# lucidrains/magvit2-pytorch

Hardware: NVIDIA H100
Metric: video-frames/sec tokenize+decode, 17x128x128 bf16 (higher is better)
Workload: dtype bf16

## Files before the change

### magvit2_pytorch_b200/csrc/tc_slab.cu

```cuda
#include "common.cuh"
#include "tc_common.cuh"
#include <cuda.h>
#include <algorithm>
#include <type_traits>
#include <mutex>
#include <map>
#include <vector>
#include <string.h>

namespace mv2 {

struct alignas(64) SlabParams {
  CUtensorMap amap;
  CUtensorMap hmap;
  CUtensorMap wmap;
  CUtensorMap wmap2;
  int kt, kh, kw, pt, ph, pw;
  int st;
  int hist_T;
  int Ci, kchunks, row_bytes;
  int B, T, H, W, Co;
  int mw, pitch, slab_h, slab_bytes, slab_stride;
  int bn, n_tiles_n, tiles_w, tiles_h, total_tiles;
  int slab_stages, w_stages;
  int tpw;
  TcEpi epi;
  int dtype;
  CUtensorMap w1map;
  const float* bias1;
  const float* se_wk;
  float se_bk;
  float* se_ws;
  CUtensorMap amap_odd;
  int dn_e_off;
  int dn_aoff[6];
  int dn_lower;
  int h_stride;
  CUtensorMap ymap;
  CUtensorMap rmap;
};

__host__ __device__ constexpr bool slab_tma_epi(int mode) {
  return mode == EPI_PLAIN || mode == EPI_PLAIN_RES || mode == EPI_GEGLU || mode == EPI_DOWN_SPACE;
}
__host__ __device__ constexpr int slab_out_box_ch(int mode, int bn, int es) {
  return (mode == EPI_GEGLU ? bn / 2 : bn) < 128 / es ? (mode == EPI_GEGLU ? bn / 2 : bn) : 128 / es;
}

__host__ __device__ __forceinline__ void slab_frame_of(const SlabParams& p, int slot, int& b, int& t) {
  const int ptc = p.pt > 0 ? (p.pt + p.st - 1) / p.st : 0;
  const int n_cheap = ptc < p.T ? ptc : p.T, n_full = p.T - n_cheap;
  const int full_slots = p.B * n_full;
  if (slot < full_slots) { b = slot / n_full; t = n_cheap + slot - b * n_full; }
  else { const int r = slot - full_slots; const int level = r / p.B; b = r - level * p.B; t = n_cheap - 1 - level; }
}
__host__ __device__ __forceinline__ int slab_tile_of_cta(const SlabParams& p, int k, int cta, int grid) {
  const int tile = k * grid + ((k & 1) ? grid - 1 - cta : cta);
  return tile < p.total_tiles ? tile : -1;
}
__device__ __forceinline__ int slab_tile_of(const SlabParams& p, int k) { return slab_tile_of_cta(p, k, blockIdx.x, gridDim.x); }

struct TileCoord { int b, t, h0, w0, n0; };
__host__ __device__ __forceinline__ TileCoord decode_tile(const SlabParams& p, int tile) {
  TileCoord c;
  const int nt = tile % p.n_tiles_n; tile /= p.n_tiles_n;
  const int tw = tile % p.tiles_w; tile /= p.tiles_w;
  const int th = tile % p.tiles_h; tile /= p.tiles_h;
  slab_frame_of(p, tile, c.b, c.t);
  c.h0 = th * 16;
  c.w0 = tw * 8 * p.mw;
  c.n0 = nt * p.bn;
  return c;
}

struct SlabSmem { uint32_t sbias, stage0, lpart, accstg, hbuf, end, rbar, otile, rtile; };
__host__ __device__ __forceinline__ SlabSmem slab_smem_layout(const SlabParams& p, uint32_t bar0, bool fused, uint32_t es) {
  SlabSmem m = {};
  m.sbias = (bar0 + 8 * (2 * p.slab_stages + 2 * p.w_stages) + 15) & ~15u;
  m.stage0 = m.sbias + (uint32_t)(p.n_tiles_n * p.bn) * 4 * (fused ? 3 : 1);
  if (fused) {
    m.lpart = m.stage0;
    m.hbuf = (m.lpart + 2048 + 1023u) & ~1023u;
    m.otile = m.hbuf + (uint32_t)p.h_stride;
    m.end = m.otile + 2u * p.mw * 64 * p.bn * es;
    return m;
  }
  m.accstg = m.stage0 + 8 * 2048;
  m.end = m.accstg + 2u * p.mw * 64 * (p.bn + 4) * 4;
  m.rbar = m.stage0;
  m.otile = (m.rbar + 32 + 1023u) & ~1023u;
  m.rtile = m.otile + 2u * p.mw * 64 * p.bn * es;
  const uint32_t tiles_end = m.rtile + (p.epi.res ? 2u * p.mw * 64 * p.bn * es : 0u);
  if (tiles_end > m.end) m.end = tiles_end;
  return m;
}

template <typename T, int MODE, int BN, int ACT>
__device__ __forceinline__ void slab_epi_mtile(const SlabParams& p, const float (&acc)[BN / 2], const TileCoord& c,
                                               const float* sbias, uint32_t ot, uint32_t rt, int wq, int lane, bool relu) {
  constexpr int ES = sizeof(T);
  constexpr int CB = slab_out_box_ch(MODE, BN, ES);
  constexpr uint32_t RB = CB * ES, BOX = 64 * RB, SWZ = (RB / 16 - 1) << 4;
  const uint32_t m0 = 16 * wq + (lane >> 2), q4 = (lane & 3) * 2 * ES;
  auto at = [&](int col, uint32_t m) {
    const uint32_t off = m * RB + (uint32_t)(col % CB) * ES + q4;
    return (uint32_t)(col / CB) * BOX + (off ^ ((off >> 3) & SWZ));
  };
  auto st2 = [](uint32_t a, float v0, float v1) {
    if constexpr (ES == 4) asm volatile("st.shared.v2.f32 [%0], {%1, %2};" ::"r"(a), "f"(v0), "f"(v1) : "memory");
    else asm volatile("st.shared.b32 [%0], %1;" ::"r"(a), "r"(pack2<T>(v0, v1)) : "memory");
  };
  const float* os = (MODE == EPI_PLAIN || MODE == EPI_PLAIN_RES) && p.epi.oscale ? p.epi.oscale + (int64_t)c.b * p.Co : nullptr;
  const float rs = MODE == EPI_PLAIN_RES && p.epi.mode == 2 ? 0.70710678118654752440f : 1.f;
  if (MODE == EPI_GEGLU) {
#pragma unroll
    for (int g = 0; g < BN / 16; ++g) {
      const int n = c.n0 + 16 * g + 2 * (lane & 3);
      const float2 bx = *reinterpret_cast<const float2*>(sbias + n), bg = *reinterpret_cast<const float2*>(sbias + n + 8);
#pragma unroll
      for (int hr = 0; hr < 2; ++hr) {
        const float* xv = &acc[8 * g + 2 * hr];
        const float* gv = &acc[8 * g + 4 + 2 * hr];
        const float v0 = gelu_fast(gv[0] + bg.x) * (xv[0] + bx.x);
        const float v1 = gelu_fast(gv[1] + bg.y) * (xv[1] + bx.y);
        st2(ot + at(8 * g, m0 + 8 * hr), v0, v1);
      }
    }
  } else {
#pragma unroll
    for (int g = 0; g < BN / 8; ++g) {
      const int col = 8 * g, n = c.n0 + col + 2 * (lane & 3);
      const float2 b = *reinterpret_cast<const float2*>(sbias + n);
      float o0 = 1.f, o1 = 1.f;
      if (os) { o0 = n < p.Co ? os[n] : 0.f; o1 = n + 1 < p.Co ? os[n + 1] : 0.f; }
#pragma unroll
      for (int hr = 0; hr < 2; ++hr) {
        float v0 = acc[4 * g + 2 * hr], v1 = acc[4 * g + 2 * hr + 1];
        if (os) { v0 *= o0; v1 *= o1; }
        v0 = act_ct<ACT>(v0 + b.x, relu);
        v1 = act_ct<ACT>(v1 + b.y, relu);
        const uint32_t a = at(col, m0 + 8 * hr);
        if (MODE == EPI_PLAIN_RES) {
          float2 rf;
          if constexpr (ES == 4) {
            asm volatile("ld.shared.v2.f32 {%0, %1}, [%2];" : "=f"(rf.x), "=f"(rf.y) : "r"(rt + a) : "memory");
          } else {
            uint32_t r;
            asm volatile("ld.shared.b32 %0, [%1];" : "=r"(r) : "r"(rt + a) : "memory");
            rf = unpack2<T>(r);
          }
          v0 = (v0 + rf.x) * rs;
          v1 = (v1 + rf.y) * rs;
        }
        st2(ot + a, v0, v1);
      }
    }
  }
}
template <typename T, int MODE, int BN, int ACT, int MWMAX>
__device__ __forceinline__ void slab_epi_fragment(const SlabParams& p, const float (&acc)[MWMAX][BN / 2], const TileCoord& c,
                                                  const float* sbias, uint32_t ot, uint32_t rt, int wq, int lane, bool relu) {
  constexpr uint32_t MTILE = (MODE == EPI_GEGLU ? BN / 2 : BN) * 64 * (int)sizeof(T);
#pragma unroll
  for (int j = 0; j < MWMAX; ++j) {
    if (j >= p.mw) break;
    slab_epi_mtile<T, MODE, BN, ACT>(p, acc[j], c, sbias, ot + j * MTILE, rt + j * MTILE, wq, lane, relu);
  }
}

constexpr int SLAB_PRODUCER_REGS = 40, SLAB_CONSUMER_REGS = 232;
template <typename T, int MODE, int BN>
__device__ __forceinline__ void tc_slab_body(const SlabParams& p) {
  constexpr int MWMAX = BN >= 32 ? 128 / BN : 4;
  constexpr int KC1 = BN >= 64 ? BN / 64 : 1;
  constexpr bool TMA_STORE = slab_tma_epi(MODE) || MODE == EPI_FUSED_RU;
  extern __shared__ uint8_t smem_raw[];
  const uint32_t smem_base = (smem_u32(smem_raw) + 1023u) & ~1023u;
  const int warp = threadIdx.x >> 5, lane = threadIdx.x & 31;
  const uint32_t row_bytes = p.row_bytes;
  const uint32_t bk = row_bytes / (uint32_t)sizeof(T);
  const uint32_t w_tile = p.bn * row_bytes;
  const uint32_t w_bytes = w_tile * p.tpw;
  const uint32_t slab0 = smem_base;
  const uint32_t wst0 = smem_base + p.slab_stages * p.slab_stride;
  const uint32_t bar0 = wst0 + p.w_stages * w_bytes;
  const uint32_t slab_full = bar0, slab_empty = slab_full + 8 * p.slab_stages;
  const uint32_t w_full = slab_empty + 8 * p.slab_stages, w_empty = w_full + 8 * p.w_stages;
  const SlabSmem L = slab_smem_layout(p, bar0, MODE == EPI_FUSED_RU, (uint32_t)sizeof(T));
  auto gen = [&](uint32_t u) { return smem_raw + (u - smem_u32(smem_raw)); };
  float* sbias = reinterpret_cast<float*>(gen(L.sbias));
  const uint32_t nbias = (uint32_t)(p.n_tiles_n * p.bn);
  const uint32_t stage0 = L.stage0;

  if (threadIdx.x == 0) {
    for (int s = 0; s < p.slab_stages; ++s) { mbar_init(slab_full + 8 * s, 1); mbar_init(slab_empty + 8 * s, 8); }
    for (int s = 0; s < p.w_stages; ++s) { mbar_init(w_full + 8 * s, 1); mbar_init(w_empty + 8 * s, 8); }
    if (MODE == EPI_PLAIN_RES)
      for (int g = 0; g < 2; ++g) { mbar_init(L.rbar + 8 * g, 1); mbar_init(L.rbar + 16 + 8 * g, 4); }
    fence_barrier_init();
  }
  if (warp == 0 && lane == 0) {
    tma_prefetch_desc(&p.amap);
    if (MODE == EPI_DOWN_SPACE) tma_prefetch_desc(&p.amap_odd);
    else if (p.hist_T > 0) tma_prefetch_desc(&p.hmap);
  }
  if (warp == 2 && lane == 0) {
    tma_prefetch_desc(&p.wmap); tma_prefetch_desc(&p.wmap2);
    if (MODE == EPI_FUSED_RU) tma_prefetch_desc(&p.w1map);
  }
  if (TMA_STORE && warp == 1 && lane == 0) {
    tma_prefetch_desc(&p.ymap);
    if (MODE == EPI_PLAIN_RES) tma_prefetch_desc(&p.rmap);
  }
  if (warp >= 4) {
    const int nb = p.n_tiles_n * p.bn;
    for (int i = threadIdx.x - 128; i < nb; i += 256) sbias[i] = (p.epi.bias && i < p.Co) ? p.epi.bias[i] : 0.f;
    if (MODE == EPI_FUSED_RU)
      for (int i = threadIdx.x - 128; i < nb; i += 256) {
        sbias[nb + i] = (p.bias1 && i < p.Co) ? p.bias1[i] : 0.f;
        sbias[2 * nb + i] = i < p.Co ? p.se_wk[i] : 0.f;
      }
  }
  __syncthreads();
  pdl_wait();
  pdl_launch_dependents();

  const int taps2d = p.kh * p.kw;

  if (warp < 4) {
    setmaxnreg_dec<SLAB_PRODUCER_REGS>();
    if (warp == 0) {
      if (MODE == EPI_DOWN_SPACE) {
        if (lane == 0) {
          uint32_t s = 0, ph = 0;
          for (int tk = 0, tile; (tile = slab_tile_of(p, tk)) >= 0; ++tk) {
            const TileCoord c = decode_tile(p, tile);
            for (int kc = 0; kc < p.kchunks; ++kc) {
              mbar_wait(slab_empty + 8 * s, ph ^ 1);
              mbar_expect_tx(slab_full + 8 * s, p.slab_bytes);
              tma_load_5d(slab0 + s * p.slab_stride, &p.amap_odd, slab_full + 8 * s, kc * bk, c.w0 - 1, c.h0 - 1, c.t, c.b);
              tma_load_5d(slab0 + s * p.slab_stride + p.dn_e_off, &p.amap, slab_full + 8 * s, kc * bk, c.w0 - 1, c.h0, c.t, c.b);
              if (++s == (uint32_t)p.slab_stages) { s = 0; ph ^= 1; }
            }
          }
        }
      } else
      if (lane == 0) {
        uint32_t s = 0, ph = 0;
        for (int tk = 0, tile; (tile = slab_tile_of(p, tk)) >= 0; ++tk) {
          const TileCoord c = decode_tile(p, tile);
          const int dt0 = max(0, p.pt - c.t * p.st - p.hist_T);
          for (int dt = dt0; dt < p.kt; ++dt)
            for (int kc = 0; kc < p.kchunks; ++kc) {
              mbar_wait(slab_empty + 8 * s, ph ^ 1);
              mbar_expect_tx(slab_full + 8 * s, p.slab_bytes);
              const int ti = c.t * p.st + dt - p.pt;
              tma_load_5d(slab0 + s * p.slab_stride, ti >= 0 ? &p.amap : &p.hmap, slab_full + 8 * s, kc * bk, c.w0 - p.pw,
                          c.h0 - p.ph, ti >= 0 ? ti : ti + p.hist_T, c.b);
              if (++s == (uint32_t)p.slab_stages) { s = 0; ph ^= 1; }
            }
        }
      }
    } else if (warp == 1) {
      if (MODE == EPI_PLAIN_RES && lane == 0) {
        constexpr int CB = slab_out_box_ch(MODE, BN, sizeof(T)), NB = BN / CB;
        constexpr uint32_t BOX = 64 * CB * (uint32_t)sizeof(T);
        uint32_t ph = 0;
        for (int tk = 0, tile; (tile = slab_tile_of(p, tk)) >= 0; ++tk) {
          const TileCoord c = decode_tile(p, tile);
          for (int g = 0; g < 2; ++g) {
            const uint32_t rt = L.rtile + (uint32_t)(g * p.mw * NB) * BOX;
            const int h = c.h0 + 8 * g;
            int nbox = 0;
            for (int j = 0; j < p.mw; ++j)
              for (int b = 0; b < NB; ++b) nbox += h < p.H && c.w0 + 8 * j < p.W && c.n0 + b * CB < p.Co;
            mbar_wait(L.rbar + 16 + 8 * g, ph ^ 1);
            mbar_expect_tx(L.rbar + 8 * g, (uint32_t)nbox * BOX);
            for (int j = 0; j < p.mw; ++j)
              for (int b = 0; b < NB; ++b)
                if (h < p.H && c.w0 + 8 * j < p.W && c.n0 + b * CB < p.Co)
                  tma_load_5d(rt + (uint32_t)(j * NB + b) * BOX, &p.rmap, L.rbar + 8 * g, c.n0 + b * CB, c.w0 + 8 * j, h, c.t, c.b);
          }
          ph ^= 1;
        }
      }
    } else if (warp == 2) {
      if (MODE == EPI_DOWN_SPACE) {
        if (lane == 0) {
          uint32_t s = 0, ph = 0;
          const int C2 = p.Ci;
          for (int tk = 0, tile; (tile = slab_tile_of(p, tk)) >= 0; ++tk) {
            const TileCoord c = decode_tile(p, tile);
            for (int kc = 0; kc < p.kchunks; ++kc)
              for (int tap = kc < p.dn_lower ? 1 : 0; tap < 6; tap += kc < p.dn_lower ? 2 : 1) {
                mbar_wait(w_empty + 8 * s, ph ^ 1);
                mbar_expect_tx(w_full + 8 * s, w_tile);
                tma_load_2d(wst0 + s * w_bytes, &p.wmap2, w_full + 8 * s, tap * C2 + kc * (int)bk, c.n0);
                if (++s == (uint32_t)p.w_stages) { s = 0; ph ^= 1; }
              }
          }
        }
      } else
      if (lane == 0) {
        uint32_t s = 0, ph = 0;
        for (int tk = 0, tile; (tile = slab_tile_of(p, tk)) >= 0; ++tk) {
          const TileCoord c = decode_tile(p, tile);
          const int dt0 = max(0, p.pt - c.t * p.st - p.hist_T);
          for (int dt = dt0; dt < p.kt; ++dt)
            for (int kc = 0; kc < p.kchunks; ++kc)
              for (int tp = 0; tp < taps2d; tp += p.tpw) {
                mbar_wait(w_empty + 8 * s, ph ^ 1);
                mbar_expect_tx(w_full + 8 * s, w_bytes);
                if (p.tpw == 1) tma_load_2d(wst0 + s * w_bytes, &p.wmap2, w_full + 8 * s, (dt * taps2d + tp) * p.Ci + kc * bk, c.n0);
                else tma_load_3d(wst0 + s * w_bytes, &p.wmap, w_full + 8 * s, kc * bk, c.n0, dt * taps2d + tp);
                if (++s == (uint32_t)p.w_stages) { s = 0; ph ^= 1; }
              }
          if (MODE == EPI_FUSED_RU)
            for (int kc2 = 0; kc2 < KC1; ++kc2) {
              mbar_wait(w_empty + 8 * s, ph ^ 1);
              mbar_expect_tx(w_full + 8 * s, w_tile);
              tma_load_2d(wst0 + s * w_bytes, &p.w1map, w_full + 8 * s, kc2 * (int)bk, 0);
              if (++s == (uint32_t)p.w_stages) { s = 0; ph ^= 1; }
            }
        }
      }
    }
  } else {
    setmaxnreg_inc<SLAB_CONSUMER_REGS>();
    const int wg = (warp - 4) >> 2, wq = warp & 3, tid = threadIdx.x & 127;
    const int sub = 2 * wg + (wq & 1), half = wq >> 1, ew = sub + 4 * half;
    const int row = sub * 32 + lane;
    const int lh = row >> 3, lw = row & 7;
    float* stg = reinterpret_cast<float*>(gen(L.accstg)) + (size_t)wg * p.mw * 64 * (BN + 4);
    const uint32_t wg_bar = 5 + wg;
    const uint32_t sbo = (uint32_t)p.pitch * row_bytes;
    const uint64_t a_hi = gmma_desc_hi(sbo, row_bytes);
    const uint64_t b_hi = gmma_desc_hi(8 * row_bytes, row_bytes);
    const bool k4 = row_bytes == 128;
    const uint32_t a_row = row_bytes >> 4;
    const uint32_t a_wg = (uint32_t)wg * 8 * (sbo >> 4);
    const uint32_t a_next_dh = (uint32_t)(p.pitch - p.kw + 1) * a_row;
    const uint32_t a_mtile = 8 * a_row;
// ... 7 lines not shown
    auto mainloop = [&](const TileCoord& c, auto mw_c, auto k4_c) {
      constexpr int MW = decltype(mw_c)::value;
      constexpr bool K4 = decltype(k4_c)::value;
      constexpr uint32_t NONE = ~0u;
      uint32_t accum = 0, pend_w = NONE, pend_s = NONE;
      auto release_pending = [&]() {
        __syncwarp();
        if (lane == 0) {
          if (pend_w != NONE) mbar_arrive(w_empty + 8 * pend_w);
          if (pend_s != NONE) mbar_arrive(slab_empty + 8 * pend_s);
        }
      };
      auto retire_previous = [&](uint32_t w_last, uint32_t s_last) {
        wgmma_wait<1>();
        release_pending();
        pend_w = w_last; pend_s = s_last;
      };
      auto next_w_stage = [&]() {
        if (++w_idx == (uint32_t)p.w_stages) { w_idx = 0; w_par ^= 1; b_lo = b_lo0; } else { b_lo += w_stage16; }
      };
      if (MODE == EPI_DOWN_SPACE) {
        for (int kc = 0; kc < p.kchunks; ++kc) {
          mbar_wait(slab_full + 8 * s_idx, s_par);
          const uint32_t a_base = desc_lo(slab0 + s_idx * p.slab_stride) + a_wg;
          const int t0 = kc < p.dn_lower ? 1 : 0, tstep = kc < p.dn_lower ? 2 : 1;
          for (int tap = t0; tap < 6; tap += tstep) {
            mbar_wait(w_full + 8 * w_idx, w_par);
            wgmma_fence();
            const uint64_t bd = b_hi | (uint64_t)b_lo;
#pragma unroll
            for (int j = 0; j < MW; ++j) {
              const uint64_t ad = a_hi | (uint64_t)(a_base + (uint32_t)p.dn_aoff[tap] + j * a_mtile);
              wgmma_mma<T, BN>(acc[j], ad, bd, accum);
              wgmma_mma<T, BN>(acc[j], ad + 2, bd + 2, 1u);
              wgmma_mma<T, BN>(acc[j], ad + 4, bd + 4, 1u);
              wgmma_mma<T, BN>(acc[j], ad + 6, bd + 6, 1u);
            }
            wgmma_commit();
            retire_previous(w_idx, tap + tstep >= 6 ? s_idx : NONE);
            accum = 1;
            next_w_stage();
          }
          if (++s_idx == (uint32_t)p.slab_stages) { s_idx = 0; s_par ^= 1; }
        }
      } else {
        const int dt0 = max(0, p.pt - c.t * p.st - p.hist_T);
        for (int dt = dt0; dt < p.kt; ++dt)
          for (int kc = 0; kc < p.kchunks; ++kc) {
            mbar_wait(slab_full + 8 * s_idx, s_par);
            uint32_t a_lo = desc_lo(slab0 + s_idx * p.slab_stride) + a_wg;
            int dw = 0;
            for (int tp0 = 0; tp0 < taps2d; tp0 += p.tpw) {
              mbar_wait(w_full + 8 * w_idx, w_par);
              const bool slab_last = tp0 + p.tpw >= taps2d;
              uint32_t b_cur = b_lo;
              for (int u = 0; u < p.tpw; ++u) {
                wgmma_fence();
                const uint64_t bd = b_hi | (uint64_t)b_cur;
#pragma unroll
                for (int j = 0; j < MW; ++j) {
                  const uint64_t ad = a_hi | (uint64_t)(a_lo + j * a_mtile);
                  wgmma_mma<T, BN>(acc[j], ad, bd, accum);
                  wgmma_mma<T, BN>(acc[j], ad + 2, bd + 2, 1u);
                  if (K4) {
                    wgmma_mma<T, BN>(acc[j], ad + 4, bd + 4, 1u);
                    wgmma_mma<T, BN>(acc[j], ad + 6, bd + 6, 1u);
                  }
                }
                wgmma_commit();
                const bool w_last = u == p.tpw - 1;
                retire_previous(w_last ? w_idx : NONE, w_last && slab_last ? s_idx : NONE);
                accum = 1;
                b_cur += w_tile16;
                if (++dw == p.kw) { dw = 0; a_lo += a_next_dh; } else { a_lo += a_row; }
              }
              next_w_stage();
            }
            if (++s_idx == (uint32_t)p.slab_stages) { s_idx = 0; s_par ^= 1; }
          }
      }
      wgmma_wait<0>();
      release_pending();
    };
    auto mainloop_k = [&](const TileCoord& c, auto mw_c) {
      if (MODE != EPI_FUSED_RU && MODE != EPI_DOWN_SPACE && !k4) mainloop(c, mw_c, std::false_type());
      else mainloop(c, mw_c, std::true_type());
    };
    for (int tk = 0, tile; (tile = slab_tile_of(p, tk)) >= 0; ++tk) {
      const TileCoord c = decode_tile(p, tile);
      if (MWMAX >= 4 && p.mw == 4) mainloop_k(c, std::integral_constant<int, (MWMAX >= 4 ? 4 : 1)>());
      else if (MWMAX >= 2 && p.mw == 2) mainloop_k(c, std::integral_constant<int, (MWMAX >= 2 ? 2 : 1)>());
      else mainloop_k(c, std::integral_constant<int, 1>());
      if (slab_tma_epi(MODE)) {
        constexpr int CB = slab_out_box_ch(MODE, BN, sizeof(T)), NB = (MODE == EPI_GEGLU ? BN / 2 : BN) / CB;
        constexpr uint32_t BOX = 64 * CB * (uint32_t)sizeof(T);
        const uint32_t ot = L.otile + (uint32_t)(wg * p.mw * NB) * BOX, rt = L.rtile + (uint32_t)(wg * p.mw) * 64 * BN * (uint32_t)sizeof(T);
        if (tid == 0) bulk_wait_read_all();
        named_bar_sync(wg_bar, 128);
        if (MODE == EPI_PLAIN_RES) mbar_wait(L.rbar + 8 * wg, r_par);
        const int act = p.epi.act;
        if (MODE == EPI_GEGLU || act == MV2_ACT_NONE)
          slab_epi_fragment<T, MODE, BN, MV2_ACT_NONE>(p, acc, c, sbias, ot, rt, wq, lane, false);
        else if (act == MV2_ACT_ELU) slab_epi_fragment<T, MODE, BN, MV2_ACT_ELU>(p, acc, c, sbias, ot, rt, wq, lane, false);
        else if (act == MV2_ACT_SILU) slab_epi_fragment<T, MODE, BN, MV2_ACT_SILU>(p, acc, c, sbias, ot, rt, wq, lane, false);
        else slab_epi_fragment<T, MODE, BN, MV2_ACT_LEAKY_RELU>(p, acc, c, sbias, ot, rt, wq, lane, act == MV2_ACT_RELU);
        if (MODE == EPI_PLAIN_RES) {
          __syncwarp();
          if (lane == 0) mbar_arrive(L.rbar + 16 + 8 * wg);
          r_par ^= 1;
        }
        fence_proxy_async();
        named_bar_sync(wg_bar, 128);
        if (tid == 0) {
          const int oc0 = MODE == EPI_GEGLU ? c.n0 / 2 : c.n0, oco = MODE == EPI_GEGLU ? p.Co / 2 : p.Co;
          const int h = c.h0 + 8 * wg;
          for (int j = 0; j < p.mw; ++j)
            for (int b = 0; b < NB; ++b)
              if (h < p.H && c.w0 + 8 * j < p.W && oc0 + b * CB < oco)
                tma_store_5d(&p.ymap, ot + (uint32_t)(j * NB + b) * BOX, oc0 + b * CB, c.w0 + 8 * j, h, c.t, c.b);
          bulk_commit();
        }
        continue;
      }
      if constexpr (MODE == EPI_FUSED_RU) {
        static_assert(sizeof(T) == 2, "the fused ResidualUnit has 16-bit instances only");
        constexpr int CB = slab_out_box_ch(MODE, BN, 2), NB = BN / CB;
        constexpr uint32_t BOX = 64 * CB * 2;
        const float* sb1 = sbias + nbias;
        const float* swk = sbias + 2 * nbias;
        float* lpart = reinterpret_cast<float*>(gen(L.lpart));
        const uint32_t hb = L.hbuf + (uint32_t)wg * KC1 * BOX, ot = L.otile + (uint32_t)(wg * p.mw * NB) * BOX;
        const int h = c.h0 + lh;
        const int rl = lane >> 2, piece = lane & 3;
        const uint32_t mrow = (uint32_t)(row & 63), mq = mrow & ~31u;
        const int recs_per_frame = p.tiles_h * p.tiles_w * 4;
        float* rec = p.se_ws + ((int64_t)(c.b * p.T + c.t) * recs_per_frame + ((c.h0 >> 4) * p.tiles_w + c.w0 / (8 * p.mw)) * 4 + sub) * (p.Co + 2);
        float run_m = -INFINITY, run_s = 0.f, run_acc[2][8];
#pragma unroll
        for (int q = 0; q < 2; ++q)
#pragma unroll
          for (int i = 0; i < 8; ++i) run_acc[q][i] = 0.f;
        const uint64_t h_hi = gmma_desc_hi(1024, 128);
        const uint32_t h_lo = desc_lo(hb);
        uint32_t w1_slot[KC1], w1_par[KC1], w1_lo[KC1];
#pragma unroll
        for (int kc2 = 0; kc2 < KC1; ++kc2) {
          w1_slot[kc2] = w_idx; w1_par[kc2] = w_par; w1_lo[kc2] = b_lo;
          if (++w_idx == (uint32_t)p.w_stages) { w_idx = 0; w_par ^= 1; b_lo = b_lo0; } else { b_lo += w_stage16; }
        }
        if (tid == 0) bulk_wait_read_all();
#pragma unroll
        for (int j = 0; j < MWMAX; ++j) {
          if (j >= p.mw) break;
          slab_epi_mtile<T, MODE, BN, MV2_ACT_ELU>(p, acc[j], c, sbias, hb, 0, wq, lane, false);
          fence_proxy_async();
          named_bar_sync(wg_bar, 128);
#pragma unroll
          for (int kc2 = 0; kc2 < KC1; ++kc2) mbar_wait(w_full + 8 * w1_slot[kc2], w1_par[kc2]);
          wgmma_fence();
#pragma unroll
          for (int kc2 = 0; kc2 < KC1; ++kc2) {
            const uint64_t ad = h_hi | (uint64_t)(h_lo + kc2 * (BOX >> 4)), bd = h_hi | (uint64_t)w1_lo[kc2];
            wgmma_mma<T, BN>(acc[0], ad, bd, kc2 > 0 ? 1u : 0u);
            wgmma_mma<T, BN>(acc[0], ad + 2, bd + 2, 1u);
            wgmma_mma<T, BN>(acc[0], ad + 4, bd + 4, 1u);
            wgmma_mma<T, BN>(acc[0], ad + 6, bd + 6, 1u);
          }
          wgmma_commit();
          wgmma_wait<0>();
          if (j == p.mw - 1) {
            __syncwarp();
            if (lane == 0)
#pragma unroll
// ... 131 lines not shown
              ks = (int64_t)4 * p.W * cy;
            } else {
              const int cy = p.Co >> 1, qd = n / cy, cb = n - qd * cy;
              yp = (T*)p.epi.y + ((((int64_t)c.b * (2 * p.T) + (2 * c.t + qd)) * p.H + h20) * p.W + w2) * cy + cb + piece * 8;
              ks = (int64_t)p.W * cy;
            }
#pragma unroll
            for (int k = 0; k < 4; ++k) {
              uint4 v;
              asm volatile("ld.shared.v4.b32 {%0, %1, %2, %3}, [%4];" : "=r"(v.x), "=r"(v.y), "=r"(v.z), "=r"(v.w)
                           : "r"(rd + k * 512 + ((piece ^ (((8 * k + rl) >> 1) & 3)) << 4)));
              if (k < klim) *reinterpret_cast<uint4*>(yp + k * ks) = v;
            }
            __syncwarp();
          }
        } else {
          for (int c0 = ((j + half) & 1) * 32; c0 < p.bn; c0 += 64) {
            uint32_t r[32];
            load_row32(srow + c0, BN < 32 ? BN : 32, r);
            if (row_ok) epi_chunk32<T, MODE>(p.epi, r, min(32, p.bn - c0), c.n0 + c0, sbias + c.n0 + c0, c.b, c.t, h, w, row_base);
          }
        }
      }
    }
    if (TMA_STORE && tid == 0) bulk_wait_all();
  }
}

template <int MODE, int BN>
__global__ void __launch_bounds__(384, 1) tc_slab_kernel(const __grid_constant__ SlabParams p) { tc_slab_body<__nv_bfloat16, MODE, BN>(p); }
template <int MODE, int BN>
__global__ void __launch_bounds__(384, 1) tc_slab_f16_kernel(const __grid_constant__ SlabParams p) { tc_slab_body<__half, MODE, BN>(p); }
template <int MODE, int BN>
__global__ void __launch_bounds__(384, 1) tc_slab_tf32_kernel(const __grid_constant__ SlabParams p) { tc_slab_body<float, MODE, BN>(p); }

}

using namespace mv2;

static bool slab_narrow(const mv2_tc_conv_args* a) { return a->out_layout == 1 && a->Co <= 16 && a->kw > 3; }

extern "C" int mv2_tc_slab_supported(const mv2_tc_conv_args* a) {
  if (!a || tc_dtype(a) < 0) return 0;
  const int ci_bytes = a->Ci * tc_esize(tc_dtype(a));
  if (a->sh != 1 || a->sw != 1) return 0;
  if (a->st != 1) {
    if (a->st != 2 || a->out_layout != 0 || a->epi_mode != 0 || a->shuffle != MV2_SHUFFLE_NONE) return 0;
    if (a->To != (a->Ti + a->pt - a->kt) / a->st + 1 || a->To < 1) return 0;
  }
  if (ci_bytes % 64 != 0 || a->Co > 4096) return 0;
  if (a->oscale && (a->epi_mode != 0 || a->shuffle != MV2_SHUFFLE_NONE)) return 0;
  if (a->epi_mode == 1 && (a->Co % 64 != 0 || a->shuffle != MV2_SHUFFLE_NONE || a->res)) return 0;
  if (a->epi_mode == 2 && (!a->res || a->shuffle != MV2_SHUFFLE_NONE)) return 0;
  if (a->epi_mode < 0 || a->epi_mode > 2) return 0;
  if (a->Co % 32 != 0 && a->Co > 32) return 0;
  if (ci_bytes % 128 != 0 && a->kw != 1) return 0;
  if (a->res && a->Co % 8 != 0) return 0;
  if (a->shuffle != MV2_SHUFFLE_NONE && ((a->shuffle == MV2_SHUFFLE_SPACE ? a->Co / 4 : a->Co / 2) % 8 != 0 || a->Co % 32 != 0)) return 0;
  if (a->kh > 7 || a->kw > (slab_narrow(a) ? 7 : 3) || a->kt > 8) return 0;
  if (a->Ho != a->Hi || a->Wo != a->Wi) return 0;
  if (a->out_layout == 1) {
    if (a->Co % 8 == 0 || a->res || a->shuffle != MV2_SHUFFLE_NONE || a->epi_mode != 0) return 0;
    if (a->To > a->Ti || a->To < 1) return 0;
    if (a->pt != a->kt - 1 - (a->Ti - a->To) && a->pt != -(a->Ti - a->To)) return 0;
  } else if (a->out_layout != 0 || (a->st == 1 && a->To != a->Ti)) return 0;
  return 1;
}

static int slab_ring_budget(const SlabParams& p, bool fused) {
  SlabParams q = p;
  q.slab_stages = 3; q.w_stages = 12;
  return 227 * 1024 - 2048 - (int)slab_smem_layout(q, 0, fused, tc_esize(p.dtype)).end;
}
static size_t slab_smem_bytes(const SlabParams& p, bool fused) {
  const uint32_t rings = (uint32_t)(p.slab_stages * p.slab_stride + p.w_stages * p.bn * p.row_bytes * p.tpw);
  return 1024 + slab_smem_layout(p, rings, fused, tc_esize(p.dtype)).end;
}
static int slab_default_mw(int bn, int Wo) { return bn <= 32 && Wo > 16 ? 4 : (bn <= 64 && Wo > 8 ? 2 : 1); }
static void slab_set_geometry(SlabParams& p, int mw) {
  p.mw = mw;
  p.pitch = 8 * mw + p.kw - 1;
  p.slab_bytes = p.pitch * p.slab_h * p.row_bytes;
  p.slab_stride = (p.slab_bytes + 1023) / 1024 * 1024;
  p.tiles_w = ceil_div(p.W, 8 * mw);
  p.total_tiles = (int)((int64_t)p.B * p.T * p.tiles_h * p.tiles_w * p.n_tiles_n);
}

static int slab_fill_plan(const mv2_tc_conv_args* a, SlabParams& p) {
  memset(&p, 0, sizeof(p));
  p.kt = a->kt; p.kh = a->kh; p.kw = a->kw; p.pt = a->pt; p.ph = a->ph; p.pw = a->pw;
  p.st = a->st;
  p.dtype = tc_dtype(a);
  const int ci_bytes = a->Ci * tc_esize(p.dtype);
  p.row_bytes = ci_bytes % 128 == 0 ? 128 : 64;
  p.Ci = a->Ci; p.kchunks = ci_bytes / p.row_bytes;
  p.B = a->B; p.T = a->To; p.H = a->Ho; p.W = a->Wo; p.Co = a->Co;
  p.epi = tc_epi_of(a);

  const int co_pad = (a->Co + 31) / 32 * 32;
  int best_bn = 32;
  for (int bn = 128; bn >= 32; bn >>= 1)
    if (co_pad % bn == 0) { best_bn = bn; break; }
  const bool ragged_ok = a->epi_mode == 0 && a->shuffle == MV2_SHUFFLE_NONE && a->Co % 8 == 0;
  if ((ragged_ok || a->epi_mode == 1) && best_bn <= 64 && co_pad >= 512 && (co_pad + 127) / 128 * 128 * 100 <= co_pad * 108)
    best_bn = 128;
  p.bn = slab_narrow(a) ? (a->Co <= 8 ? 8 : 16) : best_bn;
  p.n_tiles_n = slab_narrow(a) ? 1 : (co_pad + p.bn - 1) / p.bn;
  p.tiles_h = ceil_div(a->Ho, 16);
  p.slab_h = 16 + a->kh - 1;
  int budget;
  for (int mw = slab_default_mw(p.bn, a->Wo);; mw >>= 1) {
    slab_set_geometry(p, mw);
    budget = slab_ring_budget(p, false);
    if (mw == 1 || 2 * p.slab_stride + 2 * p.bn * p.row_bytes <= budget) break;
  }
  const int taps2d = a->kh * a->kw;
  p.tpw = 1;
  for (int d = taps2d; d >= 1; --d)
    if (taps2d % d == 0 && d * p.bn * p.row_bytes <= 32 * 1024) { p.tpw = d; break; }
  int w_bytes = p.bn * p.row_bytes * p.tpw;
  p.slab_stages = p.slab_stride * 3 + w_bytes * 3 <= budget ? 3 : 2;
  p.w_stages = std::min(12, (budget - p.slab_stages * p.slab_stride) / w_bytes);
  if (p.w_stages < 2 && p.slab_stages > 2) { p.slab_stages = 2; p.w_stages = std::min(12, (budget - 2 * p.slab_stride) / w_bytes); }
  while (p.w_stages < 2 && p.tpw > 1) {
    int d = p.tpw - 1;
    while (d > 1 && taps2d % d != 0) --d;
    p.tpw = d;
    w_bytes = p.bn * p.row_bytes * p.tpw;
    p.w_stages = std::min(12, (budget - p.slab_stages * p.slab_stride) / w_bytes);
  }
  MV2_CHECK_ARG(p.w_stages >= 2);
  return MV2_OK;
}

static int slab_encode_maps(SlabParams& p, const mv2_tc_conv_args* a, const mv2_conv_hist* hist = nullptr) {
  const CUtensorMapSwizzle swz = swizzle_of_row(p.row_bytes);
  const int es = tc_esize(p.dtype);
  const int64_t C = a->Ci, W = a->Wi, H = a->Hi, T = a->Ti;
  const cuuint64_t xdims[5] = {(cuuint64_t)C, (cuuint64_t)W, (cuuint64_t)H, (cuuint64_t)T, (cuuint64_t)a->B};
  const cuuint64_t xstrides[4] = {(cuuint64_t)(C * es), (cuuint64_t)(W * C * es), (cuuint64_t)(H * W * C * es), (cuuint64_t)(T * H * W * C * es)};
  const cuuint32_t xbox[5] = {(cuuint32_t)(p.row_bytes / es), (cuuint32_t)p.pitch, (cuuint32_t)p.slab_h, 1, 1};
  if (const int rc = encode_tc_map(&p.amap, p.dtype, 5, a->x, xdims, xstrides, xbox, swz, "slab")) return rc;
  p.hist_T = hist ? hist->T_h : 0;
  if (p.hist_T > 0) {
    const cuuint64_t hdims[5] = {(cuuint64_t)C, (cuuint64_t)W, (cuuint64_t)H, (cuuint64_t)p.hist_T, (cuuint64_t)a->B};
    const cuuint64_t hstrides[4] = {xstrides[0], xstrides[1], xstrides[2], (cuuint64_t)(hist->clip_stride * es)};
    if (const int rc = encode_tc_map(&p.hmap, p.dtype, 5, hist->h, hdims, hstrides, xbox, swz, "history")) return rc;
  }
  const int64_t ntaps = (int64_t)a->kt * a->kh * a->kw, K = ntaps * C;
  const cuuint64_t wdims[3] = {(cuuint64_t)C, (cuuint64_t)a->Co, (cuuint64_t)ntaps}, kdims[2] = {(cuuint64_t)K, (cuuint64_t)a->Co};
  const cuuint64_t wstrides[2] = {(cuuint64_t)(K * es), (cuuint64_t)(C * es)};
  const cuuint32_t wbox[3] = {(cuuint32_t)(p.row_bytes / es), (cuuint32_t)p.bn, (cuuint32_t)p.tpw};
  if (const int rc = encode_tc_map(&p.wmap, p.dtype, 3, a->w, wdims, wstrides, wbox, swz, "weights")) return rc;
  return encode_tc_map(&p.wmap2, p.dtype, 2, a->w, kdims, wstrides, wbox, swz, "weights 2-D");
}
static int slab_encode_out_maps(SlabParams& p, int mode) {
  const int es = tc_esize(p.dtype);
  const int cb = slab_out_box_ch(mode, p.bn, es);
  const int64_t oc = mode == EPI_GEGLU ? p.Co / 2 : p.Co;
  const cuuint64_t dims[5] = {(cuuint64_t)oc, (cuuint64_t)p.W, (cuuint64_t)p.H, (cuuint64_t)p.T, (cuuint64_t)p.B};
  const cuuint64_t strides[4] = {(cuuint64_t)(oc * es), (cuuint64_t)(p.W * oc * es), (cuuint64_t)(p.H * p.W * oc * es),
                                 (cuuint64_t)(p.T * p.H * p.W * oc * es)};
  const cuuint32_t box[5] = {(cuuint32_t)cb, 8, 8, 1, 1};
  const CUtensorMapSwizzle swz = swizzle_of_row(cb * es);
  if (const int rc = encode_tc_map(&p.ymap, p.dtype, 5, p.epi.y, dims, strides, box, swz, "output")) return rc;
  if (mode != EPI_PLAIN_RES) return MV2_OK;
  return encode_tc_map(&p.rmap, p.dtype, 5, p.epi.res, dims, strides, box, swz, "residual");
}

static int slab_launch(int mode, const SlabParams& p, void* stream) {
#define MV2_SLAB_BN(K, M) {K<M, 32>, K<M, 64>, K<M, 128>}
#define MV2_SLAB_NONE {nullptr, nullptr, nullptr}
#define MV2_SLAB_FLAVOURS(K, FUSED_RU, SHUFFLE_ST)                                                                       \
  {MV2_SLAB_BN(K, EPI_PLAIN), MV2_SLAB_BN(K, EPI_GEGLU), MV2_SLAB_BN(K, EPI_SHUFFLE),                                 \
   {K<EPI_RAGGED, 32>, K<EPI_RAGGED, 16>, K<EPI_RAGGED, 8>},                                                           \
   MV2_SLAB_BN(K, EPI_PLAIN_RES), FUSED_RU, SHUFFLE_ST, MV2_SLAB_BN(K, EPI_DOWN_SPACE)}
  static void (*const kernels[3][8][3])(SlabParams) = {
      MV2_SLAB_FLAVOURS(tc_slab_kernel, MV2_SLAB_BN(tc_slab_kernel, EPI_FUSED_RU), MV2_SLAB_BN(tc_slab_kernel, EPI_SHUFFLE_ST)),
      MV2_SLAB_FLAVOURS(tc_slab_f16_kernel, MV2_SLAB_BN(tc_slab_f16_kernel, EPI_FUSED_RU),
                        MV2_SLAB_BN(tc_slab_f16_kernel, EPI_SHUFFLE_ST)),
      MV2_SLAB_FLAVOURS(tc_slab_tf32_kernel, MV2_SLAB_NONE, MV2_SLAB_NONE)};
#undef MV2_SLAB_FLAVOURS
#undef MV2_SLAB_NONE
#undef MV2_SLAB_BN
  static PerDeviceOnce attr_once;
  const cudaError_t attr_err = attr_once.run([] {
    cudaError_t e = cudaSuccess;
    for (auto& type : kernels)
      for (auto& row : type)
        for (auto k : row)
          if (e == cudaSuccess && k) e = cudaFuncSetAttribute(k, cudaFuncAttributeMaxDynamicSharedMemorySize, 227 * 1024);
    return e;
  });
  if (attr_err != cudaSuccess) { set_error("cudaFuncSetAttribute failed: %s", cudaGetErrorString(attr_err)); return MV2_E_CUDA; }
  const size_t smem = slab_smem_bytes(p, mode == EPI_FUSED_RU);
  MV2_CHECK_ARG(smem <= 227 * 1024);
  int dev = 0, n_sm = 132;
  cudaGetDevice(&dev);
  cudaDeviceGetAttribute(&n_sm, cudaDevAttrMultiProcessorCount, dev);
  MV2_CHECK_ARG(p.bn >= 32 || mode == EPI_RAGGED);
  const int slot = p.bn == 32 ? 0 : (p.bn == 64 || p.bn == 16 ? 1 : 2);
  const auto kernel = kernels[p.dtype == MV2_F16 ? 1 : (p.dtype == MV2_TF32 ? 2 : 0)][mode][slot];
  MV2_CHECK_ARG(kernel != nullptr);
  launch_k(kernel, dim3(std::min(p.total_tiles, n_sm)), dim3(384), smem, (cudaStream_t)stream, p);
  MV2_CHECK_LAUNCH();
  return MV2_OK;
}

extern "C" int mv2_tc_slab_plan(const mv2_tc_conv_args* a, int n_sm, int* out6) {
  MV2_CHECK_ARG(a && out6 && n_sm > 0);
  if (!mv2_tc_slab_supported(a)) { set_error("mv2_tc_slab_plan: unsupported shape"); return MV2_E_UNSUPPORTED; }
  SlabParams p;
  if (const int rc = slab_fill_plan(a, p)) return rc;
  const int grid = std::min(p.total_tiles, n_sm);
  out6[0] = p.mw; out6[1] = p.bn; out6[2] = p.n_tiles_n; out6[3] = p.total_tiles; out6[4] = grid; out6[5] = p.slab_stages;
  return MV2_OK;
}

extern "C" int mv2_tc_slab_tile(const mv2_tc_conv_args* a, int n_sm, int cta, int k, int* out6) {
  MV2_CHECK_ARG(a && out6 && n_sm > 0 && cta >= 0 && k >= 0);
  if (!mv2_tc_slab_supported(a)) { set_error("mv2_tc_slab_tile: unsupported shape"); return MV2_E_UNSUPPORTED; }
  SlabParams p;
  if (const int rc = slab_fill_plan(a, p)) return rc;
  const int grid = std::min(p.total_tiles, n_sm);
  MV2_CHECK_ARG(cta < grid);
  const int tile = slab_tile_of_cta(p, k, cta, grid);
  out6[0] = tile;
  if (tile >= 0) {
    const TileCoord c = decode_tile(p, tile);
    out6[1] = c.b; out6[2] = c.t; out6[3] = c.h0; out6[4] = c.w0; out6[5] = c.n0;
  }
  return MV2_OK;
}

extern "C" int mv2_tc_slab_forward(const mv2_tc_conv_args* a, const mv2_conv_hist* hist, void* stream) {
  MV2_CHECK_ARG(a && a->x && a->w && a->y);
  MV2_CHECK_ARG(!hist || (hist->T_h >= 0 && (hist->T_h == 0 || (hist->h && hist->clip_stride > 0))));
  if (!mv2_tc_slab_supported(a)) { set_error("mv2_tc_slab_forward: unsupported shape"); return MV2_E_UNSUPPORTED; }
  SlabParams p;
  if (const int rc = slab_fill_plan(a, p)) return rc;
  if (const int rc = slab_encode_maps(p, a, hist)) return rc;
  int mode = EPI_PLAIN;
  if (a->epi_mode == 1) mode = EPI_GEGLU;
  else if (a->shuffle != MV2_SHUFFLE_NONE && (a->Co / (a->shuffle == MV2_SHUFFLE_SPACE ? 4 : 2)) % 32 == 0 && p.dtype != MV2_TF32)
    mode = EPI_SHUFFLE_ST;
  else if (a->shuffle != MV2_SHUFFLE_NONE) mode = EPI_SHUFFLE;
  else if (a->Co % 8 != 0) mode = EPI_RAGGED;
  else if (a->res) mode = EPI_PLAIN_RES;
  if (slab_tma_epi(mode))
    if (const int rc = slab_encode_out_maps(p, mode)) return rc;
  return slab_launch(mode, p, stream);
}


static void ru_as_conv_args(const mv2_tc_ru_args* a, mv2_tc_conv_args* c) {
  memset(c, 0, sizeof(*c));
  c->x = a->x; c->w = a->w3; c->bias = a->b3; c->res = nullptr; c->y = a->y;
  c->B = a->B; c->Ti = c->To = a->T; c->Hi = c->Ho = a->H; c->Wi = c->Wo = a->W; c->Ci = c->Co = a->C;
  c->kt = a->kt; c->kh = a->kh; c->kw = a->kw; c->st = c->sh = c->sw = 1;
  c->pt = a->kt - 1; c->ph = a->kh / 2; c->pw = a->kw / 2;
  c->act = MV2_ACT_ELU; c->shuffle = MV2_SHUFFLE_NONE; c->epi_mode = 0;
  c->dtype = a->dtype;
}

extern "C" int mv2_tc_ru_supported(const mv2_tc_ru_args* a) {
  if (!a) return 0;
  if (tc_dtype_of(a->dtype) == MV2_TF32) return 0;
  if (a->C != 64 && a->C != 128) return 0;
  if (a->W <= 8) return 0;
  if (a->kt < 1 || a->kt > 8 || a->kh < 1 || a->kh > 7 || a->kw < 1 || a->kw > 3) return 0;
  if ((a->kh & 1) == 0 || (a->kw & 1) == 0) return 0;
  mv2_tc_conv_args c;
  ru_as_conv_args(a, &c);
  return mv2_tc_slab_supported(&c);
}

static int ru_fill_plan(const mv2_tc_ru_args* a, SlabParams& p) {
  mv2_tc_conv_args c;
  ru_as_conv_args(a, &c);
  if (const int rc = slab_fill_plan(&c, p)) return rc;
  MV2_CHECK_ARG(p.bn == a->C && p.n_tiles_n == 1 && p.row_bytes == 128);
  p.tpw = 1;
  p.h_stride = p.kchunks * 16384;
  const int budget = slab_ring_budget(p, true), w_bytes = p.bn * p.row_bytes;
  p.slab_stages = 3 * p.slab_stride + 2 * w_bytes <= budget ? 3 : 2;
  p.w_stages = std::min(12, (budget - p.slab_stages * p.slab_stride) / w_bytes);
  MV2_CHECK_ARG(p.w_stages >= 2);
  p.bias1 = a->b1; p.se_wk = a->se_wk; p.se_bk = a->se_bk; p.se_ws = a->se_ws;
  return MV2_OK;
}

extern "C" int mv2_tc_ru_records(const mv2_tc_ru_args* a) {
  if (!mv2_tc_ru_supported(a)) { set_error("mv2_tc_ru_records: unsupported shape"); return MV2_E_UNSUPPORTED; }
  SlabParams p;
  if (const int rc = ru_fill_plan(a, p)) return rc;
  return p.tiles_h * p.tiles_w * 4;
}

extern "C" size_t mv2_tc_ru_workspace_bytes(const mv2_tc_ru_args* a) {
  const int recs = mv2_tc_ru_records(a);
  if (recs <= 0) return 0;
  const size_t F = (size_t)a->B * a->T;
  return (F * recs * (a->C + 2) + F * (a->C + 16)) * sizeof(float);
}

extern "C" int mv2_tc_ru_forward(const mv2_tc_ru_args* a, const mv2_conv_hist* hist, void* stream) {
  MV2_CHECK_ARG(a && a->x && a->w3 && a->w1 && a->y && a->se_wk && a->se_ws);
  MV2_CHECK_ARG(!hist || (hist->T_h >= 0 && (hist->T_h == 0 || (hist->h && hist->clip_stride > 0))));
  if (!mv2_tc_ru_supported(a)) { set_error("mv2_tc_ru_forward: unsupported shape"); return MV2_E_UNSUPPORTED; }
  SlabParams p;
  if (const int rc = ru_fill_plan(a, p)) return rc;
  mv2_tc_conv_args c;
  ru_as_conv_args(a, &c);
  if (const int rc = slab_encode_maps(p, &c, hist)) return rc;
  const cuuint64_t dims1[2] = {(cuuint64_t)a->C, (cuuint64_t)a->C};
  const cuuint64_t strides1[1] = {(cuuint64_t)a->C * 2};
  const cuuint32_t box1[2] = {64, (cuuint32_t)p.bn};
  if (const int rc = encode_tc_map(&p.w1map, p.dtype, 2, a->w1, dims1, strides1, box1, CU_TENSOR_MAP_SWIZZLE_128B, "w1")) return rc;
  if (const int rc = slab_encode_out_maps(p, EPI_FUSED_RU)) return rc;
  return slab_launch(EPI_FUSED_RU, p, stream);
}


extern "C" int mv2_tc_down_space_supported(const mv2_tc_conv_args* a) {
  if (!a || tc_dtype(a) < 0) return 0;
  const int es = tc_esize(tc_dtype(a));
  if (a->kt != 1 || a->kh != 3 || a->kw != 3 || a->st != 1 || a->sh != 2 || a->sw != 2) return 0;
  if (a->pt != 0 || a->ph != 1 || a->pw != 1) return 0;
  if ((a->Hi & 1) || (a->Wi & 1) || a->Ho != a->Hi / 2 || a->Wo != a->Wi / 2 || a->To != a->Ti) return 0;
  if ((a->Ci * es) % 128 != 0 || a->Co % 32 != 0 || a->Co > 4096) return 0;
  if (a->res || a->shuffle != MV2_SHUFFLE_NONE || a->epi_mode != 0 || a->out_layout != 0 || a->oscale) return 0;
  return 1;
}

extern "C" int mv2_tc_down_space_forward(const mv2_tc_conv_args* a, void* stream) {
  MV2_CHECK_ARG(a && a->x && a->w && a->y);
  if (!mv2_tc_down_space_supported(a)) { set_error("mv2_tc_down_space_forward: unsupported shape"); return MV2_E_UNSUPPORTED; }
  SlabParams p;
  memset(&p, 0, sizeof(p));
  p.dtype = tc_dtype(a);
  const int es = tc_esize(p.dtype);
  const int C2 = 2 * a->Ci, bk = 128 / es;
  p.kt = 1; p.kh = 3; p.kw = 2; p.pt = 0; p.ph = 1; p.pw = 1; p.st = 1;
  p.row_bytes = 128; p.Ci = C2; p.kchunks = C2 / bk; p.dn_lower = a->Ci / bk;
  p.B = a->B; p.T = a->To; p.H = a->Ho; p.W = a->Wo; p.Co = a->Co;
  p.epi = tc_epi_of(a);
  int bn = 32;
  for (int c = 128; c >= 32; c >>= 1) if (a->Co % c == 0) { bn = c; break; }
  const int w_bytes = bn * 128;
  p.bn = bn; p.n_tiles_n = a->Co / bn; p.tpw = 1;
  p.tiles_h = ceil_div(a->Ho, 16);
  p.slab_h = 17;
  int budget;
  for (int mw = slab_default_mw(bn, a->Wo);; mw >>= 1) {
    slab_set_geometry(p, mw);
    p.dn_e_off = p.slab_stride;
    const int e_bytes = 16 * p.pitch * 128;
    p.slab_bytes += e_bytes;
    p.slab_stride += (e_bytes + 1023) / 1024 * 1024;
    budget = slab_ring_budget(p, false);
    if (mw == 1 || 2 * p.slab_stride + 3 * w_bytes <= budget) break;
  }
  for (int dh = 0; dh < 3; ++dh)
// ... 22 lines not shown
```

Before: 5459.

## Batch multiple K-chunks per slab stage for 1x1 convs in tensor-core slab kernel

```diff
diff --git a/magvit2_pytorch_b200/csrc/tc_slab.cu b/magvit2_pytorch_b200/csrc/tc_slab.cu
--- a/magvit2_pytorch_b200/csrc/tc_slab.cu
+++ b/magvit2_pytorch_b200/csrc/tc_slab.cu
@@ -23,6 +23,8 @@
   int mw, pitch, slab_h, slab_bytes, slab_stride;
   int bn, n_tiles_n, tiles_w, tiles_h, total_tiles;
   int slab_stages, w_stages;
+  int kpc;
+  int tiles_only;
   int tpw;
   TcEpi epi;
   int dtype;
@@ -43,6 +45,7 @@
 __host__ __device__ constexpr bool slab_tma_epi(int mode) {
   return mode == EPI_PLAIN || mode == EPI_PLAIN_RES || mode == EPI_GEGLU || mode == EPI_DOWN_SPACE;
 }
+__host__ __device__ constexpr bool slab_kpc_mode(int mode) { return mode == EPI_PLAIN || mode == EPI_GEGLU; }
 __host__ __device__ constexpr int slab_out_box_ch(int mode, int bn, int es) {
   return (mode == EPI_GEGLU ? bn / 2 : bn) < 128 / es ? (mode == EPI_GEGLU ? bn / 2 : bn) : 128 / es;
 }
@@ -85,11 +88,13 @@
     m.end = m.otile + 2u * p.mw * 64 * p.bn * es;
     return m;
   }
-  m.accstg = m.stage0 + 8 * 2048;
-  m.end = m.accstg + 2u * p.mw * 64 * (p.bn + 4) * 4;
+  if (!p.tiles_only) {
+    m.accstg = m.stage0 + 8 * 2048;
+    m.end = m.accstg + 2u * p.mw * 64 * (p.bn + 4) * 4;
+  }
   m.rbar = m.stage0;
   m.otile = (m.rbar + 32 + 1023u) & ~1023u;
-  m.rtile = m.otile + 2u * p.mw * 64 * p.bn * es;
+  m.rtile = m.otile + 2u * p.mw * 64 * (p.epi.mode == 1 ? p.bn / 2 : p.bn) * es;
   const uint32_t tiles_end = m.rtile + (p.epi.res ? 2u * p.mw * 64 * p.bn * es : 0u);
   if (tiles_end > m.end) m.end = tiles_end;
   return m;
@@ -246,18 +251,24 @@
         }
       } else
       if (lane == 0) {
-        uint32_t s = 0, ph = 0;
+        uint32_t s = 0, ph = 0, u = 0;
+        const uint32_t chunk = (uint32_t)(p.slab_stride / p.kpc);
         for (int tk = 0, tile; (tile = slab_tile_of(p, tk)) >= 0; ++tk) {
           const TileCoord c = decode_tile(p, tile);
           const int dt0 = max(0, p.pt - c.t * p.st - p.hist_T);
           for (int dt = dt0; dt < p.kt; ++dt)
             for (int kc = 0; kc < p.kchunks; ++kc) {
-              mbar_wait(slab_empty + 8 * s, ph ^ 1);
-              mbar_expect_tx(slab_full + 8 * s, p.slab_bytes);
+              if (u == 0) {
+                mbar_wait(slab_empty + 8 * s, ph ^ 1);
+                mbar_expect_tx(slab_full + 8 * s, p.kpc * p.slab_bytes);
+              }
               const int ti = c.t * p.st + dt - p.pt;
-              tma_load_5d(slab0 + s * p.slab_stride, ti >= 0 ? &p.amap : &p.hmap, slab_full + 8 * s, kc * bk, c.w0 - p.pw,
-                          c.h0 - p.ph, ti >= 0 ? ti : ti + p.hist_T, c.b);
-              if (++s == (uint32_t)p.slab_stages) { s = 0; ph ^= 1; }
+              tma_load_5d(slab0 + s * p.slab_stride + u * chunk, ti >= 0 ? &p.amap : &p.hmap, slab_full + 8 * s, kc * bk,
+                          c.w0 - p.pw, c.h0 - p.ph, ti >= 0 ? ti : ti + p.hist_T, c.b);
+              if (++u == (uint32_t)p.kpc) {
+                u = 0;
+                if (++s == (uint32_t)p.slab_stages) { s = 0; ph ^= 1; }
+              }
             }
         }
       }
@@ -431,13 +442,50 @@
       wgmma_wait<0>();
       release_pending();
     };
+    auto mainloop_kpc = [&]() {
+      if constexpr (slab_kpc_mode(MODE)) {
+        constexpr uint32_t NONE = ~0u;
+        const uint32_t chunk16 = (uint32_t)(p.slab_stride / p.kpc) >> 4;
+        uint32_t accum = 0, pend_w = NONE, pend_s = NONE;
+        auto release_pending = [&]() {
+          __syncwarp();
+          if (lane == 0) {
+            if (pend_w != NONE) mbar_arrive(w_empty + 8 * pend_w);
+            if (pend_s != NONE) mbar_arrive(slab_empty + 8 * pend_s);
+          }
+        };
+        for (int kc = 0; kc < p.kchunks; kc += p.kpc) {
+          mbar_wait(slab_full + 8 * s_idx, s_par);
+          uint32_t a_lo = desc_lo(slab0 + s_idx * p.slab_stride) + a_wg;
+          for (int u = 0; u < p.kpc; ++u, a_lo += chunk16) {
+            mbar_wait(w_full + 8 * w_idx, w_par);
+            wgmma_fence();
+            const uint64_t ad = a_hi | (uint64_t)a_lo, bd = b_hi | (uint64_t)b_lo;
+            wgmma_mma<T, BN>(acc[0], ad, bd, accum);
+            wgmma_mma<T, BN>(acc[0], ad + 2, bd + 2, 1u);
+            wgmma_mma<T, BN>(acc[0], ad + 4, bd + 4, 1u);
+            wgmma_mma<T, BN>(acc[0], ad + 6, bd + 6, 1u);
+            wgmma_commit();
+            wgmma_wait<1>();
+            release_pending();
+            pend_w = w_idx; pend_s = u == p.kpc - 1 ? s_idx : NONE;
+            accum = 1;
+            if (++w_idx == (uint32_t)p.w_stages) { w_idx = 0; w_par ^= 1; b_lo = b_lo0; } else { b_lo += w_stage16; }
+          }
+          if (++s_idx == (uint32_t)p.slab_stages) { s_idx = 0; s_par ^= 1; }
+        }
+        wgmma_wait<0>();
+        release_pending();
+      }
+    };
     auto mainloop_k = [&](const TileCoord& c, auto mw_c) {
       if (MODE != EPI_FUSED_RU && MODE != EPI_DOWN_SPACE && !k4) mainloop(c, mw_c, std::false_type());
       else mainloop(c, mw_c, std::true_type());
     };
     for (int tk = 0, tile; (tile = slab_tile_of(p, tk)) >= 0; ++tk) {
       const TileCoord c = decode_tile(p, tile);
-      if (MWMAX >= 4 && p.mw == 4) mainloop_k(c, std::integral_constant<int, (MWMAX >= 4 ? 4 : 1)>());
+      if (slab_kpc_mode(MODE) && p.kpc > 1) mainloop_kpc();
+      else if (MWMAX >= 4 && p.mw == 4) mainloop_k(c, std::integral_constant<int, (MWMAX >= 4 ? 4 : 1)>());
       else if (MWMAX >= 2 && p.mw == 2) mainloop_k(c, std::integral_constant<int, (MWMAX >= 2 ? 2 : 1)>());
       else mainloop_k(c, std::integral_constant<int, 1>());
       if (slab_tma_epi(MODE)) {
@@ -735,11 +783,23 @@
   p.pitch = 8 * mw + p.kw - 1;
   p.slab_bytes = p.pitch * p.slab_h * p.row_bytes;
   p.slab_stride = (p.slab_bytes + 1023) / 1024 * 1024;
+  p.kpc = 1;
   p.tiles_w = ceil_div(p.W, 8 * mw);
   p.total_tiles = (int)((int64_t)p.B * p.T * p.tiles_h * p.tiles_w * p.n_tiles_n);
 }
 
-static int slab_fill_plan(const mv2_tc_conv_args* a, SlabParams& p) {
+static int slab_mode_of(const mv2_tc_conv_args* a, int dtype) {
+  if (a->epi_mode == 1) return EPI_GEGLU;
+  if (a->shuffle != MV2_SHUFFLE_NONE && (a->Co / (a->shuffle == MV2_SHUFFLE_SPACE ? 4 : 2)) % 32 == 0 && dtype != MV2_TF32)
+    return EPI_SHUFFLE_ST;
+  if (a->shuffle != MV2_SHUFFLE_NONE) return EPI_SHUFFLE;
+  if (a->Co % 8 != 0) return EPI_RAGGED;
+  return a->res ? EPI_PLAIN_RES : EPI_PLAIN;
+}
+
+constexpr int SLAB_KPC_MIN_W_STAGES = 5;
+
+static int slab_fill_plan(const mv2_tc_conv_args* a, SlabParams& p, bool fused = false) {
   memset(&p, 0, sizeof(p));
   p.kt = a->kt; p.kh = a->kh; p.kw = a->kw; p.pt = a->pt; p.ph = a->ph; p.pw = a->pw;
   p.st = a->st;
@@ -781,6 +841,21 @@
     p.tpw = d;
     w_bytes = p.bn * p.row_bytes * p.tpw;
     p.w_stages = std::min(12, (budget - p.slab_stages * p.slab_stride) / w_bytes);
+  }
+  const int mode = slab_mode_of(a, p.dtype);
+  if (!fused && a->kt * taps2d == 1 && a->pt == 0 && slab_kpc_mode(mode) && p.mw == 1 && p.row_bytes == 128) {
+    SlabParams q = p;
+    q.tiles_only = 1;
+    const int budget1 = slab_ring_budget(q, false), chunk = p.slab_stride;
+    for (int kpc = 4; kpc >= 2; kpc >>= 1)
+      if (p.kchunks % kpc == 0 && p.kchunks >= 2 * kpc &&
+          p.slab_stages * kpc * chunk + SLAB_KPC_MIN_W_STAGES * w_bytes <= budget1) {
+        p.tiles_only = 1;
+        p.kpc = kpc;
+        p.slab_stride = kpc * chunk;
+        p.w_stages = std::min(12, (budget1 - p.slab_stages * p.slab_stride) / w_bytes);
+        break;
+      }
   }
   MV2_CHECK_ARG(p.w_stages >= 2);
   return MV2_OK;
@@ -893,13 +968,7 @@
   SlabParams p;
   if (const int rc = slab_fill_plan(a, p)) return rc;
   if (const int rc = slab_encode_maps(p, a, hist)) return rc;
-  int mode = EPI_PLAIN;
-  if (a->epi_mode == 1) mode = EPI_GEGLU;
-  else if (a->shuffle != MV2_SHUFFLE_NONE && (a->Co / (a->shuffle == MV2_SHUFFLE_SPACE ? 4 : 2)) % 32 == 0 && p.dtype != MV2_TF32)
-    mode = EPI_SHUFFLE_ST;
-  else if (a->shuffle != MV2_SHUFFLE_NONE) mode = EPI_SHUFFLE;
-  else if (a->Co % 8 != 0) mode = EPI_RAGGED;
-  else if (a->res) mode = EPI_PLAIN_RES;
+  const int mode = slab_mode_of(a, p.dtype);
   if (slab_tma_epi(mode))
     if (const int rc = slab_encode_out_maps(p, mode)) return rc;
   return slab_launch(mode, p, stream);
@@ -931,7 +1000,7 @@
 static int ru_fill_plan(const mv2_tc_ru_args* a, SlabParams& p) {
   mv2_tc_conv_args c;
   ru_as_conv_args(a, &c);
-  if (const int rc = slab_fill_plan(&c, p)) return rc;
+  if (const int rc = slab_fill_plan(&c, p, true)) return rc;
   MV2_CHECK_ARG(p.bn == a->C && p.n_tiles_n == 1 && p.row_bytes == 128);
   p.tpw = 1;
   p.h_stride = p.kchunks * 16384;
```

Result: no change. 5486, median of 6 (+0.5%).
